# Hansard-T/FHE-Linformer

Measured on AMD Instinct MI355X. Metric: encrypted Linformer-d128 forward ms/sample, lower is better.
Workload: dtype u64

## Files before the change

### fhe-linformer_amd/csrc/context.cpp

```cpp
#include "context.h"
#include <hip/hip_runtime.h>
#include <algorithm>
#include <cstdio>
#include <cstdlib>
#include <cstring>
#include <sys/random.h>
#include <time.h>
#include <cxxabi.h>
#include <dlfcn.h>
#include <execinfo.h>

namespace fhelin {

template <class T>
const T* Context::upload_table(const std::vector<T>& v) {
    void* p = nullptr;
    size_t bytes = std::max<size_t>(v.size() * sizeof(T), 16);
    hip_check(hipMalloc(&p, bytes), "hipMalloc(table)");
    if (!v.empty()) hip_check(hipMemcpy(p, v.data(), v.size() * sizeof(T), hipMemcpyHostToDevice), "hipMemcpy(table)");
    table_allocs.push_back(p);
    return static_cast<const T*>(p);
}
template const u64* Context::upload_table<u64>(const std::vector<u64>&);
template const int* Context::upload_table<int>(const std::vector<int>&);
// ... 53 lines not shown
    try {
        chain = make_prime_chain(p.log_n, p.n_q, p.first_bits, p.scale_bits, p.n_p, p.special_bits);
    } catch (const std::exception& e) {
        throw Error(FHELIN_ERR_ARG, std::string("prime chain: ") + e.what());
    }
    moduli = chain.q;
    moduli.insert(moduli.end(), chain.p.begin(), chain.p.end());
    for (u64 q : moduli)
        if (q >> 60) throw Error(FHELIN_ERR_ARG, "prime chain: a modulus is >= 2^60 (lower scale_bits or first_bits)");
    for (u64 q : moduli) {
        barrett.push_back(h_barrett(q));
        tw.push_back(make_twiddles(q, p.log_n));
    }
    sf_real.assign(p.n_q + 1, 0.0L);
    sf_real[0] = (long double)chain.q[L];
    for (int k = 0; k < L; ++k) sf_real[k + 1] = sf_real[k] * sf_real[k] / (long double)chain.q[L - k];

    pool.fill_word = DevicePool::parse_fill(std::getenv("FHELIN_POOL_FILL"));

    if (p.device < 0) return;

    int ndev = 0;
    if (hipGetDeviceCount(&ndev) != hipSuccess || ndev <= 0)
        throw Error(FHELIN_ERR_NO_DEVICE, "no HIP device visible: the fhe-linformer_amd engine has no CPU fallback");
    if (p.device >= ndev) throw Error(FHELIN_ERR_ARG, "device index out of range");
    hip_check(hipSetDevice(p.device), "hipSetDevice");
    hip_check(hipStreamCreateWithFlags(&stream, hipStreamNonBlocking), "hipStreamCreate");
    main_stream = stream;
    own_stream = true;
    {
        int want = 2;
        if (const char* e = std::getenv("FHELIN_LANES")) want = std::atoi(e);
        n_lanes = std::max(0, std::min(want, DevicePool::MAX_LANES - 1));
        for (int k = 1; k <= n_lanes; ++k) {
            hip_check(hipStreamCreateWithFlags(&lane_stream[k], hipStreamNonBlocking), "hipStreamCreate(lane)");
            hip_check(hipEventCreateWithFlags(&lane_event[k], hipEventDisableTiming), "hipEventCreate(lane)");
        }
        hip_check(hipEventCreateWithFlags(&fork_event, hipEventDisableTiming), "hipEventCreate(fork)");
        pool.lane_stream[0] = main_stream;
        for (int k = 1; k <= n_lanes; ++k) pool.lane_stream[k] = lane_stream[k];
        pool.have_streams = true;
        if (const char* e = std::getenv("FHELIN_ASYNC")) async_lanes = std::atoi(e) != 0;
        if (const char* e = std::getenv("FHELIN_FUSE_MODDOWN")) fuse_moddown = std::atoi(e) != 0;
        if (const char* e = std::getenv("FHELIN_FUSE_FINISH")) fuse_finish = std::atoi(e) != 0;
        if (const char* e = std::getenv("FHELIN_HOST_ENCODE")) host_encode = std::atoi(e) != 0;
        if (const char* e = std::getenv("FHELIN_DEVICE_DECODE")) device_decode = std::atoi(e) != 0;
        if (const char* e = std::getenv("FHELIN_ROT_GATHER")) rot_gather = std::atoi(e) != 0;
        if (const char* e = std::getenv("FHELIN_FUSE_LIFT")) fuse_lift = std::atoi(e) != 0;
        if (const char* e = std::getenv("FHELIN_LDS_DIGITS")) lds_digits = std::atoi(e) != 0;
        if (const char* e = std::getenv("FHELIN_FUSE_ACCP_ROWS")) fuse_accp_rows = std::atoi(e);
        if (const char* e = std::getenv("FHELIN_ACCP_ROWS_MIN_VECS")) accp_rows_min_vecs = std::atoi(e);
        if (const char* e = std::getenv("FHELIN_FUSE_ACCQ_ROWS")) fuse_accq_rows = std::atoi(e);
        if (const char* e = std::getenv("FHELIN_ACCQ_ROWS_MIN_VECS")) accq_rows_min_vecs = std::atoi(e);
        if (const char* e = std::getenv("FHELIN_NTT_TRACE")) trace_small_ntt = std::atoi(e);
        if (const char* e = std::getenv("FHELIN_SCALAR_TRACE")) trace_scalar = std::atoi(e);
        if (const char* e = std::getenv("FHELIN_HOST_WAITS")) trace_waits = std::atoi(e) != 0;
    }
    hip_check(hipEventCreate(&ev_start), "hipEventCreate");
    stage_words = (size_t)2 << p.log_n;
    for (int i = 0; i < STAGE_SLOTS; ++i) {
        hip_check(hipHostMalloc(reinterpret_cast<void**>(&stage_buf[i]), stage_words * sizeof(u64), hipHostMallocDefault), "hipHostMalloc(stage)");
        hip_check(hipEventCreateWithFlags(&stage_ev[i], hipEventDisableTiming), "hipEventCreate(stage)");
    }
    hip_check(hipHostMalloc(reinterpret_cast<void**>(&small_buf), (size_t)SMALL_SLOTS * SMALL_WORDS * sizeof(u64), hipHostMallocDefault), "hipHostMalloc(stage, small)");
    for (int i = 0; i < SMALL_SLOTS; ++i) hip_check(hipEventCreateWithFlags(&small_ev[i], hipEventDisableTiming), "hipEventCreate(stage, small)");
    hip_check(hipEventCreate(&ev_stop), "hipEventCreate");
    has_device = true;

    const int nl = (int)moduli.size();
    {
        std::vector<u64> bar(2 * nl), ninv(8 * nl, 0);
        for (int i = 0; i < nl; ++i) {
            bar[2 * i] = barrett[i].r0;
            bar[2 * i + 1] = barrett[i].r1;
            ninv[8 * i] = tw[i].n_inv;
            ninv[8 * i + 1] = tw[i].n_inv_s;
            ninv[8 * i + 2] = tw[i].w1_n_inv;
            ninv[8 * i + 3] = tw[i].w1_n_inv_s;
            int bits = 0;
            while (bits < 64 && (moduli[i] >> bits)) ++bits;
            if (bits >= 12 && bits <= 60) {
                ninv[8 * i + 4] = (u64)(bits - 10);
                ninv[8 * i + 5] = (u64)((((u128)1) << (bits + 22)) / moduli[i]);
            }
        }
        dt.log_n = p.log_n;
        dt.n_limbs = nl;
        dt.moduli = upload_table(moduli);
        dt.barrett = upload_table(bar);
        {
            std::vector<u64> qi(nl);
            for (int i = 0; i < nl; ++i) {
                u64 x = moduli[i];
                for (int it = 0; it < 6; ++it) x *= 2 - moduli[i] * x;
                qi[i] = x;
            }
            dt.qinv = upload_table(qi);
            std::vector<u64> mr(2 * (size_t)nl);
            for (int i = 0; i < nl; ++i) {
                mr[2 * i] = mont_r(moduli[i]);
                mr[2 * i + 1] = h_shoup(mr[2 * i], moduli[i]);
            }
            dt.mont = upload_table(mr);
        }
        dt.ninv = upload_table(ninv);
        std::vector<u64> f((size_t)nl * 2 * N), g((size_t)nl * 2 * N);
// ... 337 lines not shown
```

### fhe-linformer_amd/csrc/context.h

```cpp
#pragma once
#include <cstdint>
#include <map>
#include <memory>
#include <stdexcept>
#include <string>
#include <unordered_map>
#include <vector>
#include <hip/hip_runtime_api.h>
#include "../../include/fhelin.h"
#include "hostmath.h"
#include "pool.h"
#include "kernels_elem.h"

namespace fhelin {

struct Params {
    int log_n = 16;
    int n_q = 24;
    int first_bits = 55;
    int scale_bits = 52;
    int n_p = 6;
    int special_bits = 60;
    int dnum = 4;
    int log_slots = 14;
// ... 85 lines not shown
    u64* small_buf = nullptr;
    hipEvent_t small_ev[SMALL_SLOTS] = {};
    bool small_used[SMALL_SLOTS] = {};
    int small_next = 0;
    void upload_async(u64* dst, const u64* src, size_t words);

    const u64* d_phatinv = nullptr;
    const u64* d_phatmod = nullptr;
    const u64* d_pinv = nullptr;
    const u64* d_pmod = nullptr;
    const u64* d_qlinv = nullptr;
    const u64* d_qlmod = nullptr;
    std::vector<LevelTables> lvl;
    std::map<u64, const u32*> automorph_maps;

    explicit Context(const Params& p);
    ~Context();
    Context(const Context&) = delete;
    Context& operator=(const Context&) = delete;

    void require_device() const;
    template <class T> T* dalloc(size_t count) { return static_cast<T*>(pool.alloc(count * sizeof(T))); }
    template <class T> Scratch<T> scratch(size_t count) { return Scratch<T>(pool, count); }
    template <class T> const T* upload_table(const std::vector<T>& v);
    int limb_id_q(int i) const { return i; }
    int limb_id_p(int j) const { return L + 1 + j; }
    int digits_at(int ell) const { return (ell + alpha - 1) / alpha; }
    u64 galois_element(long rot_index) const;
    int stride = 1;
    bool stride_explicit = false;
    bool stride_locked = false;
    u64 rot_element(int rot_index) const { return stride == 1 ? galois_element(rot_index) : galois_element((long)stride * rot_index); }
    struct PhysicalScope {
        Context& c;
        int was;
        explicit PhysicalScope(Context& ctx) : c(ctx), was(ctx.stride) { c.stride = 1; }
        ~PhysicalScope() { c.stride = was; }
    };
    const u32* automorph_map(u64 galois);
    const u32* automorph_inverse_of(const u32* map);
    std::map<const u32*, const u32*> automorph_inverse;
    u32 automorph_ginv_of(const u32* map) const;
    std::map<const u32*, u32> automorph_ginv;
    bool fuse_finish = true;
    bool fuse_moddown = false;
    bool host_encode = false;
    bool device_decode = false;
    bool rot_gather = true;
    bool fuse_lift = true;
    int fuse_accp_rows = 1;
    int accp_rows_min_vecs = 0;
    int fuse_accq_rows = 1;
    int accq_rows_min_vecs = 0;
    bool lds_digits = true;
    struct FftDev {
        const u32* rot = nullptr;
        const double* ksi = nullptr;
    };
    std::map<int, FftDev> fft_dev;
    void sync();
    void ntt(const LimbBatch& b, bool inverse, int active = -1) {
        stats.limb_ntt += (u64)(active >= 0 ? active : b.nvec);
        if (trace_small_ntt && b.nvec <= trace_small_ntt) note_small_ntt(b.nvec);
        launch_ntt(dt, b, inverse, stream);
    }
    bool trace_waits = false;
    std::map<std::string, std::pair<u64, u64>> wait_sites;
    void note_wait(const char* site, u64 ns) {
        auto& e = wait_sites[site];
        e.first += 1;
        e.second += ns;
    }
    int trace_small_ntt = 0;
    std::map<std::string, std::pair<u64, u64>> small_ntt_sites;
    void note_small_ntt(int nvec);
    int trace_scalar = 0;
    std::map<std::string, std::pair<u64, u64>> scalar_sites;
    void note_scalar(int nvec);
    void ntt_epilogue(const LimbBatch& b, const NttEpilogue& ep) {
        stats.limb_ntt += (u64)b.nvec;
        if (trace_small_ntt && b.nvec <= trace_small_ntt) note_small_ntt(b.nvec);
        launch_ntt_epilogue(dt, b, ep, stream);
    }
    void ntt_epilogue_product(const LimbBatch& b, const NttEpilogue& ep, const NttProduct& p) {
        stats.limb_ntt += (u64)b.nvec;
        if (trace_small_ntt && b.nvec <= trace_small_ntt) note_small_ntt(b.nvec);
        launch_ntt_epilogue_product(dt, b, ep, p, stream);
    }
};

}
```

### fhe-linformer_amd/csrc/evaluator.cpp

```cpp
#include "evaluator.h"
#include <map>
#include <hip/hip_runtime.h>
#include <cmath>
#include <cstring>

namespace fhelin {

DevBlock::~DevBlock() {
    if (d && ctx) {
        try { ctx->pool.free(d); } catch (...) {}
    }
}
Ciphertext::~Ciphertext() {
    if (async_ev) (void)hipEventDestroy(async_ev);
    if (d && ctx && !block) {
        try { ctx->pool.free(d); } catch (...) {}
    }
}
Encoding::~Encoding() {
    if (ready) (void)hipEventDestroy(ready);
    if (d && ctx) {
        try { ctx->pool.free(d, lanes_ordered); } catch (...) {}
    }
}
// ... 131 lines not shown
}

void Evaluator::keyswitch(const u64* c_ntt, int ell, const EvalKey& key, u64* out, const u64* add0, const u64* add1,
                          const u32* map, const u64* post) {
    keyswitch_batch(1, c_ntt, 0, ell, key, out, 0, add0, add1, 0, map, post, 0);
}

void Evaluator::keyswitch_batch(int B, const u64* c_ntt, size_t c_stride, int ell, const EvalKey& key, u64* out, size_t out_stride,
                                const u64* add0, const u64* add1, size_t add_stride, const u32* map, const u64* post,
                                size_t post_stride) {
    keyswitch_impl(B, nullptr, c_ntt, c_stride, ell, &key, out, out_stride, add0, add1, add_stride, map, post, post_stride);
}

void Evaluator::keyswitch_rows(const KsRows& rows, const u64* c_ntt, size_t c_stride, int ell, u64* out, size_t out_stride,
                               const u64* add0, size_t add_stride) {
    const int B = (int)rows.keys.size();
    if (B < 1) return;
    if (B > KsShape::MAX_ROWS || rows.maps.size() != rows.keys.size()) throw Error(FHELIN_ERR_ARG, "keyswitch_rows: bad row count");
    keyswitch_impl(B, &rows, c_ntt, c_stride, ell, nullptr, out, out_stride, add0, nullptr, add_stride, nullptr, nullptr, 0);
}

void Evaluator::keyswitch_impl(int B, const KsRows* rows, const u64* c_ntt, size_t c_stride, int ell, const EvalKey* key, u64* out,
                               size_t out_stride, const u64* add0, const u64* add1, size_t add_stride, const u32* map, const u64* post,
                               size_t post_stride) {
    c_.require_device();
    if (c_.K < 1) throw Error(FHELIN_ERR_STATE, "hybrid key switching needs at least one special prime");
    if (B < 1) return;
    KsShape sh = ks_shape(ell, B, {c_stride, out_stride, add_stride, post_stride});
    const bool shared = rows && rows->shared_input;
    if (rows) {
        sh.per_row = 1;
        sh.shared_input = shared ? 1 : 0;
        for (int b = 0; b < B; ++b) {
            sh.evk_row[b] = rows->keys[b]->d;
            sh.map_row[b] = rows->maps[b];
        }
    }
    KsShape shu = sh;
    shu.batch = shared ? 1 : B;
    c_.stats.keyswitch += (u64)B;
    c_.stats.keyswitch_limbs += (u64)B * ell;
    const bool identity = !map && !rows;
    const bool gather = !identity && !add1 && rot_in_gather();
    const u64* evk = key ? key->d : nullptr;
    if (gather) evk = set_gather(sh, rows ? rows->keys.data() : &key, rows ? rows->maps.data() : &map, add0, add_stride);
    Scratch<u64> ext = modup(shu, c_ntt, !gather);
    KsAcc acc = inner_product(sh, ext, evk, c_ntt, moddown_tail(gather ? KsOutput::Gathered : identity ? KsOutput::Identity : KsOutput::Scattered));
    moddown(acc, gather ? KsOut{out, nullptr, nullptr, post} : KsOut{out, add0, add1, post, map});
    launch_ok("keyswitch");
}


KsShape Evaluator::ks_shape(int ell, int batch, const KsStrides& st) const {
    return KsShape{ell, c_.K, c_.alpha, c_.lvl[ell].beta, c_.L + 1, batch, st.c, st.out, st.add, st.post};
}

Evaluator::KsTail Evaluator::moddown_tail(KsOutput o) const {
    const bool rows = o == KsOutput::Gathered || (o == KsOutput::Identity && (c_.fuse_moddown || c_.fuse_finish)) ||
                      (o == KsOutput::Scattered && c_.fuse_moddown) || (o == KsOutput::MergedSum && c_.fuse_finish && c_.rot_gather);
    return rows ? KsTail::RowPass : KsTail::Finish;
}

const u64* Evaluator::set_gather(KsShape& sh, const EvalKey* const* keys, const u32* const* maps, const u64* c0, size_t c0_stride) {
    const u64* evk = nullptr;
    sh.gather = 1;
    if (sh.per_row) {
        for (int b = 0; b < (sh.row_mod ? sh.row_mod : sh.batch); ++b) {
            sh.evk_row[b] = permuted(*keys[b], maps[b]);
            sh.ginv_row[b] = c_.automorph_ginv_of(maps[b]);
        }
    } else {
        evk = permuted(*keys[0], maps[0]);
        sh.map_row[0] = maps[0];
        sh.ginv = c_.automorph_ginv_of(maps[0]);
    }
    if (c0) {
        sh.gsrc = c0;
        sh.gsrc_stride = c0_stride;
        sh.gsrc_pmod = c_.d_pmod;
    }
    return evk;
}

Scratch<u64> Evaluator::modup(const KsShape& up, const u64* src, bool times_r2, int group2, size_t group2_stride) {
    const size_t N = c_.N;
    const int n = up.batch, ell = up.ell, nt = ell + c_.K;
    const LevelTables& lt = c_.lvl[ell];
    Scratch<u64> cc = c_.scratch<u64>((size_t)n * ell * N);
    {
        LimbBatch ib{cc, n * ell, nullptr, 0, ell, src};
        if (n > 1 && up.c_stride != (size_t)ell * N) {
            ib.src_group = ell;
            ib.src_group_stride = up.c_stride;
        }
        if (group2 > 0) {
            ib.src_group2 = group2;
            ib.src_group2_stride = group2_stride;
        }
        c_.ntt(ib, true);
    }
    Scratch<u64> ext = c_.scratch<u64>((size_t)n * lt.beta * nt * N);
    launch_modup_conv(c_.dt, up, ext, cc, src, lt.up_hatinv, times_r2 ? lt.up_hatmod_r2 : lt.up_hatmod, c_.stream);
    LimbBatch eb{ext, n * lt.beta * nt, lt.ext_limb_tab, 0, 1};
    eb.tab_len = lt.beta * nt;
    eb.lazy_out = true;
    c_.ntt(eb, false, n * (lt.beta * nt - ell));
    return ext;
// ... 1875 lines not shown
```

### fhe-linformer_amd/csrc/kernels_elem.h

```cpp
#pragma once
#include "kernels.h"

namespace fhelin {

struct ScalarSet {
    u64 v[128];
};

void launch_ew_mul(const DeviceTables& t, u64* out, const u64* a, const u64* b, int nvec, int b_mod, int limb_first, int limb_count, hipStream_t s);
void launch_ew_add(const DeviceTables& t, u64* out, const u64* a, const u64* b, int nvec, int b_mod, int limb_first, int limb_count, hipStream_t s);
void launch_ew_sub(const DeviceTables& t, u64* out, const u64* a, const u64* b, int nvec, int b_mod, int limb_first, int limb_count, hipStream_t s);
void launch_ew_muladd(const DeviceTables& t, u64* out, const u64* acc, const u64* a, const u64* b, int nvec, int b_mod, int limb_first,
                      int limb_count, hipStream_t s);
void launch_ew_neg(const DeviceTables& t, u64* out, const u64* a, int nvec, int limb_first, int limb_count, hipStream_t s);
void launch_ew_scalar(const DeviceTables& t, u64* out, const u64* a, const ScalarSet& sc, int nvec, int limb_first, int limb_count, hipStream_t s,
                      int in_limbs = 0);
void launch_ew_addscalar(const DeviceTables& t, u64* out, const u64* a, const ScalarSet& sc, int nvec, int limb_first, int limb_count, hipStream_t s,
                         int add_vecs = -1);
struct LinComb {
    static constexpr int MAX_TERMS = 32;
    int n = 0;
    int vecs = 0;
    const u64* a[MAX_TERMS];
};
// ... 81 lines not shown
};
void launch_ew_dot_groups(const DeviceTables& t, const EwDotGroups& d, hipStream_t s);
struct EwCyclic {
    static constexpr int PERIOD = 32;
    int n = 0, ell = 0;
    const u64* a[PERIOD];
    const u64* m[PERIOD];
    u64* out[PERIOD];
};
void launch_ew_cyclic_dot(const DeviceTables& t, const EwCyclic& d, hipStream_t s);
struct EwWindow {
    static constexpr int W = 32;
    int ell = 0, accumulate = 0;
    u32 cur_mask = 0, prev_mask = 0;
    const u64* cur[W];
    const u64* prev[W];
    const u64* m[W];
    u64* out[W];
};
void launch_ew_window_dot(const DeviceTables& t, const EwWindow& d, hipStream_t s);

struct KsShape {
    int ell;
    int k;
    int alpha;
    int beta;
    int L1;
    int batch = 1;
    size_t c_stride = 0;
    size_t out_stride = 0;
    size_t add_stride = 0;
    size_t post_stride = 0;
    static constexpr int MAX_ROWS = 16;
    int per_row = 0;
    int shared_input = 0;
    int row_mod = 0;
    const u64* evk_row[MAX_ROWS] = {};
    const u32* map_row[MAX_ROWS] = {};
    static constexpr int MAX_ROT = 7;
    int n_rot = 0;
    const u64* evk_rot[MAX_ROT] = {};
    const u32* map_rot[MAX_ROT] = {};
    size_t rot_ext_stride = 0;
    size_t rot_input_stride = 0;
    int lds_digits = 0;
    size_t ext_batch_stride = 0;
    const u64* gsrc = nullptr;
    size_t gsrc_stride = 0;
    const u64* gsrc_pmod = nullptr;
    int gather = 0;
    u32 ginv = 0;
    u32 ginv_row[MAX_ROWS] = {};
    int tch = 16;
    int accp_limbs = 0;
    int accp_rows = 0;
    int accq_rows = 0;
};
struct NttProduct {
    KsShape sh;
    const u64* ext = nullptr;
    const u64* evk = nullptr;
    int multi = 0;
    const u64* c_ntt = nullptr;
};
void launch_ntt_rows_product(const DeviceTables& t, const LimbBatch& b, const NttProduct& p, hipStream_t s);
void launch_ntt_epilogue_product(const DeviceTables& t, const LimbBatch& b, const NttEpilogue& ep, const NttProduct& p, hipStream_t s);
void launch_ntt_cols_inverse(const DeviceTables& t, const LimbBatch& b, hipStream_t s);
void launch_modup_conv(const DeviceTables& t, const KsShape& sh, u64* ext, const u64* cc, const u64* c_ntt, const u64* hatinv,
                       const u64* hatmod, hipStream_t s);
void launch_ks_inner(const DeviceTables& t, const KsShape& sh, u64* accQ, u64* accP, const u64* ext, const u64* evk, const u64* c_ntt,
                     hipStream_t s);
void launch_ks_inner_multi(const DeviceTables& t, const KsShape& sh, u64* accQ, u64* accP, const u64* ext, const u64* c_ntt,
                           hipStream_t s);
void launch_fold_key(const DeviceTables& t, u64* out, const u64* key, const u32* map, const u64* V, int nvec, hipStream_t s);
struct HoistAdd {
    int n_rot = 0;
    const u64* v[KsShape::MAX_ROT + 1] = {};
    const u32* map[KsShape::MAX_ROT] = {};
    u64* acc = nullptr;
    const u64* pmod = nullptr;
};
void launch_hoist_addends(const DeviceTables& t, const KsShape& sh, const HoistAdd& h, u64* pre, const u64* ct, hipStream_t s);
struct LtStep {
    static constexpr int MAX_G = 4;
    const u64* key;
    const u32* map;
    const u64* v[MAX_G];
    u32 mask;
    u32 pad;
};
struct LtDot {
    static constexpr int MAX_STEPS = 32;
    const LtStep* steps = nullptr;
    int n_steps = 0;
    int n_groups = 0;
    int g0 = 0, groups = 0;
    const u64* pmod = nullptr;
};
void launch_ks_inner_dot(const DeviceTables& t, const KsShape& sh, const LtDot& ld, u64* accQ, u64* accP, const u64* ext, const u64* c0,
                         const u64* c1, hipStream_t s);
void launch_moddown_conv(const DeviceTables& t, const KsShape& sh, u64* conv, const u64* accP, const u64* phatinv, const u64* phatmod,
                         hipStream_t s);
void launch_affine_acc(const DeviceTables& t, const KsShape& sh, u64* accQ, const u64* d, const u64* sub, const ScalarSet& cst, int has_cst, int f,
                       const u64* pmod, hipStream_t s);
void launch_moddown_rescale_conv(const DeviceTables& t, const KsShape& sh, u64* conv, const u64* accP, const u64* top, const u64* hatinv,
                                 const u64* hatmod, const u64* mmod, hipStream_t s);
// ... 16 lines not shown
```

### fhe-linformer_amd/csrc/kernels_ks.hip

```cpp
#include <hip/hip_runtime.h>
#include <cstdlib>
#include "kernels.h"
#include "kernels_elem.h"

namespace fhelin {
namespace {

typedef u64 u64x2 __attribute__((ext_vector_type(2)));

__device__ __forceinline__ Barrett load_barrett(const DeviceTables& t, int limb) {
    Barrett b;
    b.q = t.moduli[limb];
    b.r0 = t.barrett[2 * limb];
    b.r1 = t.barrett[2 * limb + 1];
    return b;
}

constexpr int TCH = 16;

template <int MAXA, bool FULL>
__device__ __forceinline__ void modup_body(const DeviceTables& t, const KsShape& sh, u64* __restrict__ ext, const u64* __restrict__ cc,
                                           const u64* __restrict__ hatinv, const u64* __restrict__ hatmod, int j, int lo, int cnt, size_t n) {
    const size_t N = (size_t)1 << t.log_n;
    const int nt = sh.ell + sh.k;
    u32 y0[MAXA], y1[MAXA];
#pragma unroll
    for (int i = 0; i < MAXA; ++i) {
        if (FULL || i < cnt) {
            const int li = lo + i;
            split30(mul_shoup(cc[(size_t)li * N + n], hatinv[2 * li], hatinv[2 * li + 1], t.moduli[li]), y0[i], y1[i]);
        } else {
            y0[i] = y1[i] = 0;
        }
    }
    u64* dst = ext + (size_t)j * nt * N + n;
    const int t0 = blockIdx.z * sh.tch, t1 = min(nt, t0 + sh.tch);
    for (int tt = t0; tt < t1; ++tt) {
        if (tt >= lo && tt < lo + cnt) continue;
        const int limb = tt < sh.ell ? tt : sh.L1 + (tt - sh.ell);
        const u64 qt = t.moduli[limb], qti = t.qinv[limb];
        u64 slo = 0, shi = 0;
#pragma unroll
        for (int i0 = 0; i0 < MAXA; i0 += 8) {
            Acc30 acc = {0, 0, 0};
#pragma unroll
            for (int i = i0; i < i0 + 8 && i < MAXA; ++i)
                if (FULL || i < cnt) {
                    const u64 h = hatmod[(size_t)(lo + i) * nt + tt];
                    mac30(acc, y0[i], y1[i], (u32)h, (u32)(h >> 32));
                }
            acc30_flush(acc, slo, shi);
        }
        dst[(size_t)tt * N] = redc128(slo, shi, qt, qti);
    }
}

template <int MAXA>
__global__ __launch_bounds__(256) void modup_conv_kernel(DeviceTables t, KsShape sh, u64* __restrict__ ext, const u64* __restrict__ cc, const u64* __restrict__ c_ntt,
                                                         const u64* __restrict__ hatinv, const u64* __restrict__ hatmod) {
    const int bi = blockIdx.y / sh.beta, j = blockIdx.y % sh.beta;
    const size_t N = (size_t)1 << t.log_n;
    const size_t n = (size_t)blockIdx.x * 256 + threadIdx.x;
    const int lo = j * sh.alpha;
    const int cnt = min(sh.alpha, sh.ell - lo);
    const int nt = sh.ell + sh.k;
    cc += (size_t)bi * sh.ell * N;
    ext += (size_t)bi * sh.beta * nt * N;
    (void)c_ntt;
    if (cnt == MAXA)
        modup_body<MAXA, true>(t, sh, ext, cc, hatinv, hatmod, j, lo, cnt, n);
    else
        modup_body<MAXA, false>(t, sh, ext, cc, hatinv, hatmod, j, lo, cnt, n);
}

struct KsBlock {
    int bx, bi, tt;
};
__device__ __forceinline__ KsBlock ks_block(const KsShape& sh, int rows = 0) {
    const unsigned nx = gridDim.x, nblk = gridDim.x * gridDim.y;
    const unsigned nb = rows ? (unsigned)rows : (unsigned)sh.batch;
    unsigned b = blockIdx.y * nx + blockIdx.x;
    if ((nblk & 7) == 0) b = (b & 7) * (nblk >> 3) + (b >> 3);
    KsBlock k;
    k.bi = (int)(b % nb);
    k.bx = (int)((b / nb) % nx);
    k.tt = (int)(b / (nb * nx));
    return k;
}

__device__ __forceinline__ u32 sel_mask(u32 a, u32 b, unsigned long long mask) {
    u32 r;
    asm("v_cndmask_b32_e64 %0, %1, %2, %3" : "=v"(r) : "v"(a), "v"(b), "s"(mask));
    return r;
}

template <bool GATHER>
__global__ __launch_bounds__(256) void ks_inner_kernel(DeviceTables t, KsShape sh, u64* __restrict__ accQ, u64* __restrict__ accP, const u64* __restrict__ ext,
                                                       const u64* __restrict__ evk, const u64* __restrict__ c_ntt) {
    const int nt = sh.ell + sh.k;
    const KsBlock kb_ = ks_block(sh);
    const int bi = kb_.bi, tt = kb_.tt;
    const int limb = tt < sh.ell ? tt : sh.L1 + (tt - sh.ell);
    const int in = sh.row_mod ? bi / sh.row_mod : bi;
    const int ri = sh.per_row ? (sh.row_mod ? bi % sh.row_mod : bi) : 0;
    if (sh.row_mod) {
        ext += (size_t)in * sh.ext_batch_stride;
        c_ntt += (size_t)in * sh.c_stride;
        evk = sh.evk_row[bi % sh.row_mod];
    } else {
        if (!sh.shared_input) {
            ext += (size_t)bi * sh.beta * nt * ((size_t)1 << t.log_n);
            c_ntt += (size_t)bi * sh.c_stride;
        }
        if (sh.per_row) evk = sh.evk_row[bi];
    }
    const int own = tt < sh.ell ? tt / sh.alpha : -1;
    accQ += (size_t)bi * 2 * sh.ell * ((size_t)1 << t.log_n);
    const int pk = sh.accp_limbs ? sh.accp_limbs : sh.k;
    accP += (size_t)bi * 2 * pk * ((size_t)1 << t.log_n);
    const Barrett br = load_barrett(t, limb);
    const size_t row = ((size_t)1 << t.log_n) >> 1;
    const size_t n2 = (size_t)kb_.bx * 256 + threadIdx.x;
    const size_t kstride = (size_t)(sh.L1 + sh.k) * row;
    const u64x2* E = reinterpret_cast<const u64x2*>(ext);
    const u64x2* K = reinterpret_cast<const u64x2*>(evk);
// ... 363 lines not shown
    u32 z0[MAXK], z1[MAXK];
#pragma unroll
    for (int p = 0; p < MAXK; ++p) {
        if (FULL || p < sh.k) {
            const u64 m = t.moduli[sh.L1 + p];
            u64 x = accP[((size_t)c * sh.k + p) * N + n];
            if constexpr (SIGNED) x = neg && x ? m - x : x;
            split30(mul_shoup(x, phatinv[2 * p], phatinv[2 * p + 1], m), z0[p], z1[p]);
        } else {
            z0[p] = z1[p] = 0;
        }
    }
    u64* dst = conv + (size_t)c * sh.ell * N + n;
    const int t0 = blockIdx.z * sh.tch, t1 = min(sh.ell, t0 + sh.tch);
    for (int tt = t0; tt < t1; ++tt) {
        const u64 qt = t.moduli[tt], qti = t.qinv[tt];
        u64 slo = 0, shi = 0;
#pragma unroll
        for (int p0 = 0; p0 < MAXK; p0 += 8) {
            Acc30 acc = {0, 0, 0};
#pragma unroll
            for (int p = p0; p < p0 + 8 && p < MAXK; ++p)
                if (FULL || p < sh.k) {
                    const u64 h = phatmod[(size_t)p * sh.L1 + tt];
                    mac30(acc, z0[p], z1[p], (u32)h, (u32)(h >> 32));
                }
            acc30_flush(acc, slo, shi);
        }
        u64 r = redc128(slo, shi, qt, qti);
        if constexpr (SIGNED) r = neg && r ? qt - r : r;
        dst[(size_t)tt * N] = r;
    }
}

template <int MAXK, bool SIGNED = false>
__global__ __launch_bounds__(256) void moddown_conv_kernel(DeviceTables t, KsShape sh, u64* __restrict__ conv, const u64* __restrict__ accP, const u64* __restrict__ phatinv,
                                                           const u64* __restrict__ phatmod) {
    const int bi = blockIdx.y >> 1, c = blockIdx.y & 1;
    const size_t N = (size_t)1 << t.log_n;
    const size_t n = (size_t)blockIdx.x * 256 + threadIdx.x;
    accP += (size_t)bi * 2 * sh.k * N;
    conv += (size_t)bi * 2 * sh.ell * N;
    bool neg = false;
    if constexpr (SIGNED) {
        const u32 gi = sh.per_row ? sh.ginv_row[sh.row_mod ? bi % sh.row_mod : bi] : sh.ginv;
        neg = ((gi * (u32)n) & (u32)(2 * N - 1)) >= (u32)N;
    }
    if (sh.k == MAXK)
        moddown_body<MAXK, true, SIGNED>(t, sh, conv, accP, phatinv, phatmod, c, n, neg);
    else
        moddown_body<MAXK, false, SIGNED>(t, sh, conv, accP, phatinv, phatmod, c, n, neg);
}

__global__ __launch_bounds__(256) void moddown_finish_kernel(DeviceTables t, KsShape sh, u64* __restrict__ out, const u64* __restrict__ accQ, const u64* __restrict__ conv,
                                                             const u64* __restrict__ pinv, const u64* __restrict__ add0, const u64* __restrict__ add1, const u32* __restrict__ map,
                                                             const u64* __restrict__ post) {
    const int bi = blockIdx.y / (2 * sh.ell), v = blockIdx.y % (2 * sh.ell);
    const int c = v / sh.ell, tt = v % sh.ell;
    const u64 q = t.moduli[tt];
    const u64 w = pinv[2 * tt], ws = pinv[2 * tt + 1];
    const size_t N = (size_t)1 << t.log_n;
    const size_t j = ((size_t)blockIdx.x * 256 + threadIdx.x) * 2;
    accQ += (size_t)bi * 2 * sh.ell * N;
    conv += (size_t)bi * 2 * sh.ell * N;
    out += (size_t)bi * sh.out_stride;
    const u64* add = c == 0 ? add0 : add1;
    if (add) add += (size_t)(sh.row_mod ? bi / sh.row_mod : bi) * sh.add_stride;
    if (post) post += (size_t)bi * sh.post_stride;
    if (sh.per_row) map = sh.map_row[sh.row_mod ? bi % sh.row_mod : bi];
    u64x2 r;
    if (map) {
        const u32 m0 = map[j], m1 = map[j + 1];
        r.x = mul_shoup(sub_mod(accQ[(size_t)v * N + m0], conv[(size_t)v * N + m0], q), w, ws, q);
        r.y = mul_shoup(sub_mod(accQ[(size_t)v * N + m1], conv[(size_t)v * N + m1], q), w, ws, q);
        if (add) {
            r.x = add_mod(r.x, add[(size_t)tt * N + m0], q);
            r.y = add_mod(r.y, add[(size_t)tt * N + m1], q);
        }
    } else {
        const u64x2 a = reinterpret_cast<const u64x2*>(accQ)[((size_t)v * N + j) >> 1];
        const u64x2 b = reinterpret_cast<const u64x2*>(conv)[((size_t)v * N + j) >> 1];
        r.x = mul_shoup(sub_mod(a.x, b.x, q), w, ws, q);
        r.y = mul_shoup(sub_mod(a.y, b.y, q), w, ws, q);
        if (add) {
            const u64x2 d = reinterpret_cast<const u64x2*>(add)[((size_t)tt * N + j) >> 1];
            r.x = add_mod(r.x, d.x, q);
            r.y = add_mod(r.y, d.y, q);
        }
    }
    if (post) {
        const u64x2 p = reinterpret_cast<const u64x2*>(post)[((size_t)v * N + j) >> 1];
        r.x = add_mod(r.x, p.x, q);
        r.y = add_mod(r.y, p.y, q);
    }
    if (sh.gsrc && !sh.gsrc_pmod && c == 0) {
        const u64* __restrict__ g = sh.gsrc + (size_t)bi * sh.gsrc_stride + (size_t)tt * N;
        for (int rr = 0; rr < sh.n_rot; ++rr) {
            const u64* __restrict__ gr = g + (size_t)rr * sh.rot_input_stride;
            const u32* __restrict__ mr = sh.map_rot[rr];
            const u32 m0 = mr ? mr[j] : (u32)j;
            const u64x2 gp = reinterpret_cast<const u64x2*>(gr)[m0 >> 1];
            r.x = add_mod(r.x, (m0 & 1) ? gp.y : gp.x, q);
            r.y = add_mod(r.y, (m0 & 1) ? gp.x : gp.y, q);
        }
    }
    reinterpret_cast<u64x2*>(out)[((size_t)v * N + j) >> 1] = r;
// ... 219 lines not shown
                                                                         const u64* __restrict__ phatmod, const u64* __restrict__ pinv,
                                                                         const u64* __restrict__ pmod, const u64* __restrict__ qlm) {
    const int bi = blockIdx.y >> 1;
    const size_t N = (size_t)1 << t.log_n;
    const size_t n = (size_t)blockIdx.x * 256 + threadIdx.x;
    const bool f2 = (f2_mask >> bi) & 1;
    const u64* src = accP + (size_t)blockIdx.y * (sh.k + 1) * N + n;
    u64* dst = conv + (size_t)blockIdx.y * (sh.ell - 1) * N + n;
    if (sh.k == MAXK)
        moddown_exact_body<MAXK, true>(t, sh, f2, dst, src, phatinv, phatmod, pinv, pmod, qlm);
    else
        moddown_exact_body<MAXK, false>(t, sh, f2, dst, src, phatinv, phatmod, pinv, pmod, qlm);
}

__global__ __launch_bounds__(256) void moddown_rescale_finish_kernel(DeviceTables t, KsShape sh, u64* __restrict__ out, const u64* __restrict__ accQ,
                                                                     const u64* __restrict__ conv, const u64* __restrict__ minv) {
    const int e1 = sh.ell - 1;
    const int bi = blockIdx.y / (2 * e1), v = blockIdx.y % (2 * e1);
    const int c = v / e1, tt = v % e1;
    const u64 q = t.moduli[tt];
    const u64 w = minv[2 * tt], ws = minv[2 * tt + 1];
    const size_t row = ((size_t)1 << t.log_n) >> 1;
    const size_t n2 = (size_t)blockIdx.x * 256 + threadIdx.x;
    const u64x2 a = reinterpret_cast<const u64x2*>(accQ)[(((size_t)bi * 2 + c) * sh.ell + tt) * row + n2];
    const u64x2 b = reinterpret_cast<const u64x2*>(conv)[(((size_t)bi * 2 + c) * e1 + tt) * row + n2];
    u64x2 r;
    r.x = mul_shoup(sub_mod(a.x, b.x, q), w, ws, q);
    r.y = mul_shoup(sub_mod(a.y, b.y, q), w, ws, q);
    reinterpret_cast<u64x2*>(out + (size_t)bi * sh.out_stride)[(size_t)v * row + n2] = r;
}

}

void launch_fold_key(const DeviceTables& t, u64* out, const u64* key, const u32* map, const u64* V, int nvec, hipStream_t s) {
    hipLaunchKernelGGL(fold_key_kernel, dim3((1u << t.log_n) / 512, (unsigned)nvec), dim3(256), 0, s, t, out, key, map, V);
}
void launch_hoist_addends(const DeviceTables& t, const KsShape& sh, const HoistAdd& h, u64* pre, const u64* ct, hipStream_t s) {
    hipLaunchKernelGGL(hoist_addends_kernel, dim3((1u << t.log_n) / 512, (unsigned)(sh.batch * 2 * sh.ell)), dim3(256), 0, s, t, sh, h, pre, ct);
}

void launch_affine_acc(const DeviceTables& t, const KsShape& sh, u64* accQ, const u64* d, const u64* sub, const ScalarSet& cst, int has_cst, int f,
                       const u64* pmod, hipStream_t s) {
    hipLaunchKernelGGL(affine_acc_kernel, dim3((1u << t.log_n) / 512, (unsigned)(sh.batch * 2 * sh.ell)), dim3(256), 0, s, t, sh, accQ, d, sub, cst,
                       has_cst, f, pmod);
}
static int conv_tch(unsigned planes, int targets) {
    static const int force = [] {
        const char* e = std::getenv("FHELIN_CONV_CHUNKS");
        return e ? std::atoi(e) : 0;
    }();
    if (force || planes < 2048u) return TCH;
    return targets > TCH ? targets : TCH;
}
void launch_moddown_rescale_conv(const DeviceTables& t, const KsShape& sh_in, u64* conv, const u64* accP, const u64* top, const u64* hatinv,
                                 const u64* hatmod, const u64* mmod, hipStream_t s) {
    KsShape sh = sh_in;
    const unsigned nx = (1u << t.log_n) / 256;
    sh.tch = conv_tch(nx * (unsigned)(sh.batch * 2), sh.ell - 1);
    dim3 g(nx, (unsigned)(sh.batch * 2), (unsigned)((sh.ell - 1 + sh.tch - 1) / sh.tch));
    hipLaunchKernelGGL(moddown_rescale_conv_kernel, g, dim3(256), 0, s, t, sh, conv, accP, top, hatinv, hatmod, mmod);
}
void launch_affine_acc_items(const DeviceTables& t, const KsShape& sh, const AffineItems& it, u64* accQ, u64* accP, const u64* d,
                             const u64* consts, const u64* pmod, hipStream_t s) {
    dim3 g((1u << t.log_n) / 512, (unsigned)(sh.batch * 2 * sh.ell));
    hipLaunchKernelGGL(affine_acc_items_kernel, g, dim3(256), 0, s, t, sh, it, accQ, accP, d, consts, pmod);
}
void launch_moddown_rescale_exact_conv(const DeviceTables& t, const KsShape& sh_in, u32 f2, u64* conv, const u64* accP, const u64* phatinv,
                                       const u64* phatmod, const u64* pinv, const u64* pmod, const u64* qlm, hipStream_t s) {
    KsShape sh = sh_in;
    const unsigned nx = (1u << t.log_n) / 256;
    sh.tch = conv_tch(nx * (unsigned)(sh.batch * 2), sh.ell - 1);
    dim3 g(nx, (unsigned)(sh.batch * 2), (unsigned)((sh.ell - 1 + sh.tch - 1) / sh.tch));
#define FHELIN_MDX_CASE(K) case K: hipLaunchKernelGGL((moddown_rescale_exact_conv_kernel<K>), g, dim3(256), 0, s, t, sh, f2, conv, accP, phatinv, phatmod, pinv, pmod, qlm); break;
    switch (sh.k) {
        FHELIN_MDX_CASE(1) FHELIN_MDX_CASE(2) FHELIN_MDX_CASE(3) FHELIN_MDX_CASE(4)
        FHELIN_MDX_CASE(5) FHELIN_MDX_CASE(6) FHELIN_MDX_CASE(7) FHELIN_MDX_CASE(8)
        default: hipLaunchKernelGGL((moddown_rescale_exact_conv_kernel<16>), g, dim3(256), 0, s, t, sh, f2, conv, accP, phatinv, phatmod, pinv, pmod, qlm); break;
    }
#undef FHELIN_MDX_CASE
}
void launch_moddown_rescale_finish(const DeviceTables& t, const KsShape& sh, u64* out, const u64* accQ, const u64* conv, const u64* minv,
                                   hipStream_t s) {
    dim3 g((1u << t.log_n) / 512, (unsigned)(sh.batch * 2 * (sh.ell - 1)));
    hipLaunchKernelGGL(moddown_rescale_finish_kernel, g, dim3(256), 0, s, t, sh, out, accQ, conv, minv);
}

void launch_modup_conv(const DeviceTables& t, const KsShape& sh_in, u64* ext, const u64* cc, const u64* c_ntt, const u64* hatinv,
                       const u64* hatmod, hipStream_t s) {
    KsShape sh = sh_in;
    const unsigned nx = (1u << t.log_n) / 256;
    sh.tch = conv_tch(nx * (unsigned)(sh.batch * sh.beta), sh.ell + sh.k);
    dim3 g(nx, (unsigned)(sh.batch * sh.beta), (unsigned)((sh.ell + sh.k + sh.tch - 1) / sh.tch));
#define FHELIN_MODUP_CASE(A) case A: hipLaunchKernelGGL((modup_conv_kernel<A>), g, dim3(256), 0, s, t, sh, ext, cc, c_ntt, hatinv, hatmod); break;
    switch (sh.alpha) {
        FHELIN_MODUP_CASE(1) FHELIN_MODUP_CASE(2) FHELIN_MODUP_CASE(3) FHELIN_MODUP_CASE(4)
        FHELIN_MODUP_CASE(5) FHELIN_MODUP_CASE(6) FHELIN_MODUP_CASE(7) FHELIN_MODUP_CASE(8)
        default: hipLaunchKernelGGL((modup_conv_kernel<16>), g, dim3(256), 0, s, t, sh, ext, cc, c_ntt, hatinv, hatmod); break;
    }
#undef FHELIN_MODUP_CASE
}
void launch_ks_inner(const DeviceTables& t, const KsShape& sh, u64* accQ, u64* accP, const u64* ext, const u64* evk, const u64* c_ntt,
                     hipStream_t s) {
    dim3 g((1u << t.log_n) / 512, (unsigned)(sh.batch * (sh.accp_rows ? sh.ell : sh.ell + sh.k)));
    if (sh.gather)
        hipLaunchKernelGGL(ks_inner_kernel<true>, g, dim3(256), 0, s, t, sh, accQ, accP, ext, evk, c_ntt);
    else
        hipLaunchKernelGGL(ks_inner_kernel<false>, g, dim3(256), 0, s, t, sh, accQ, accP, ext, evk, c_ntt);
}
void launch_ks_inner_multi(const DeviceTables& t, const KsShape& sh, u64* accQ, u64* accP, const u64* ext, const u64* c_ntt,
                           hipStream_t s) {
    static const int pair_rows = [] { const char* e = std::getenv("FHELIN_KS_ROW_PAIRS"); return e ? std::atoi(e) : 1; }();
    const bool stage = sh.lds_digits && sh.rot_ext_stride == 0 && sh.beta <= 4;
    const int nt = sh.accp_rows ? sh.ell : sh.ell + sh.k;
    if (pair_rows && sh.batch >= 2) {
        dim3 g((1u << t.log_n) / 512, (unsigned)(((sh.batch + 1) / 2) * nt));
        if (stage)
            hipLaunchKernelGGL((ks_inner_multi_kernel<true, 2>), g, dim3(256), 0, s, t, sh, accQ, accP, ext, c_ntt);
        else
            hipLaunchKernelGGL((ks_inner_multi_kernel<false, 2>), g, dim3(256), 0, s, t, sh, accQ, accP, ext, c_ntt);
        return;
    }
    dim3 g((1u << t.log_n) / 512, (unsigned)(sh.batch * nt));
    if (stage)
        hipLaunchKernelGGL((ks_inner_multi_kernel<true, 1>), g, dim3(256), 0, s, t, sh, accQ, accP, ext, c_ntt);
    else
        hipLaunchKernelGGL((ks_inner_multi_kernel<false, 1>), g, dim3(256), 0, s, t, sh, accQ, accP, ext, c_ntt);
}
void launch_ks_inner_dot(const DeviceTables& t, const KsShape& sh, const LtDot& ld, u64* accQ, u64* accP, const u64* ext, const u64* c0,
                         const u64* c1, hipStream_t s) {
    dim3 g((1u << t.log_n) / 512, (unsigned)(sh.batch * (sh.ell + sh.k)));
    if (ld.n_groups == 1)
        hipLaunchKernelGGL(ks_inner_dot_kernel<1>, g, dim3(256), 0, s, t, sh, ld, accQ, accP, ext, c0, c1);
    else if (ld.n_groups == 2)
        hipLaunchKernelGGL(ks_inner_dot_kernel<2>, g, dim3(256), 0, s, t, sh, ld, accQ, accP, ext, c0, c1);
    else
        hipLaunchKernelGGL((ks_inner_dot_kernel<LtStep::MAX_G>), g, dim3(256), 0, s, t, sh, ld, accQ, accP, ext, c0, c1);
}
void launch_moddown_conv(const DeviceTables& t, const KsShape& sh_in, u64* conv, const u64* accP, const u64* phatinv, const u64* phatmod,
                         hipStream_t s) {
    KsShape sh = sh_in;
    const unsigned nx = (1u << t.log_n) / 256;
    sh.tch = conv_tch(nx * (unsigned)(2 * sh.batch), sh.ell);
    dim3 g(nx, (unsigned)(2 * sh.batch), (unsigned)((sh.ell + sh.tch - 1) / sh.tch));
#define FHELIN_MODDOWN_CASE(K, S) case K: hipLaunchKernelGGL((moddown_conv_kernel<K, S>), g, dim3(256), 0, s, t, sh, conv, accP, phatinv, phatmod); break;
#define FHELIN_MODDOWN_SWITCH(S)                                                                                                                \
    switch (sh.k) {                                                                                                                             \
        FHELIN_MODDOWN_CASE(1, S) FHELIN_MODDOWN_CASE(2, S) FHELIN_MODDOWN_CASE(3, S) FHELIN_MODDOWN_CASE(4, S)                                 \
        FHELIN_MODDOWN_CASE(5, S) FHELIN_MODDOWN_CASE(6, S) FHELIN_MODDOWN_CASE(7, S) FHELIN_MODDOWN_CASE(8, S)                                 \
        default: hipLaunchKernelGGL((moddown_conv_kernel<16, S>), g, dim3(256), 0, s, t, sh, conv, accP, phatinv, phatmod); break;              \
    }
    if (sh.gather) {
        FHELIN_MODDOWN_SWITCH(true)
    } else {
        FHELIN_MODDOWN_SWITCH(false)
    }
#undef FHELIN_MODDOWN_SWITCH
#undef FHELIN_MODDOWN_CASE
}
void launch_moddown_finish(const DeviceTables& t, const KsShape& sh, u64* out, const u64* accQ, const u64* conv, const u64* pinv,
                           const u64* add0, const u64* add1, const u32* map, const u64* post, hipStream_t s) {
    dim3 g((1u << t.log_n) / 512, (unsigned)(sh.batch * 2 * sh.ell));
    hipLaunchKernelGGL(moddown_finish_kernel, g, dim3(256), 0, s, t, sh, out, accQ, conv, pinv, add0, add1, map, post);
}

}
```

Before: 216.9.

## Process two coefficients per thread in modup and moddown base conversion kernels

Adds pair variants of the modup and moddown base-conversion kernels. Each thread loads two adjacent coefficients as a 128-bit vector and reuses each target modulus's constants and hatmod row for both, halving the grid's x dimension. Constants for the next target are prefetched while the current one is computed. The pair path is on by default when alpha or k is at most 8 and the buffers are 16-byte aligned. This cuts per-coefficient table loads and widens memory accesses, at the cost of more registers per thread and possibly lower occupancy.

```diff
diff --git a/fhe-linformer_amd/csrc/context.cpp b/fhe-linformer_amd/csrc/context.cpp
--- a/fhe-linformer_amd/csrc/context.cpp
+++ b/fhe-linformer_amd/csrc/context.cpp
@@ -129,6 +129,7 @@
         if (const char* e = std::getenv("FHELIN_ACCP_ROWS_MIN_VECS")) accp_rows_min_vecs = std::atoi(e);
         if (const char* e = std::getenv("FHELIN_FUSE_ACCQ_ROWS")) fuse_accq_rows = std::atoi(e);
         if (const char* e = std::getenv("FHELIN_ACCQ_ROWS_MIN_VECS")) accq_rows_min_vecs = std::atoi(e);
+        if (const char* e = std::getenv("FHELIN_CONV_PAIRS")) conv_pairs = std::atoi(e) != 0;
         if (const char* e = std::getenv("FHELIN_NTT_TRACE")) trace_small_ntt = std::atoi(e);
         if (const char* e = std::getenv("FHELIN_SCALAR_TRACE")) trace_scalar = std::atoi(e);
         if (const char* e = std::getenv("FHELIN_HOST_WAITS")) trace_waits = std::atoi(e) != 0;
diff --git a/fhe-linformer_amd/csrc/context.h b/fhe-linformer_amd/csrc/context.h
--- a/fhe-linformer_amd/csrc/context.h
+++ b/fhe-linformer_amd/csrc/context.h
@@ -161,6 +161,7 @@
     int accp_rows_min_vecs = 0;
     int fuse_accq_rows = 1;
     int accq_rows_min_vecs = 0;
+    bool conv_pairs = true;
     bool lds_digits = true;
     struct FftDev {
         const u32* rot = nullptr;
diff --git a/fhe-linformer_amd/csrc/evaluator.cpp b/fhe-linformer_amd/csrc/evaluator.cpp
--- a/fhe-linformer_amd/csrc/evaluator.cpp
+++ b/fhe-linformer_amd/csrc/evaluator.cpp
@@ -207,7 +207,9 @@
 
 
 KsShape Evaluator::ks_shape(int ell, int batch, const KsStrides& st) const {
-    return KsShape{ell, c_.K, c_.alpha, c_.lvl[ell].beta, c_.L + 1, batch, st.c, st.out, st.add, st.post};
+    KsShape sh{ell, c_.K, c_.alpha, c_.lvl[ell].beta, c_.L + 1, batch, st.c, st.out, st.add, st.post};
+    sh.conv_pairs = c_.conv_pairs ? 1 : 0;
+    return sh;
 }
 
 Evaluator::KsTail Evaluator::moddown_tail(KsOutput o) const {
diff --git a/fhe-linformer_amd/csrc/kernels_elem.h b/fhe-linformer_amd/csrc/kernels_elem.h
--- a/fhe-linformer_amd/csrc/kernels_elem.h
+++ b/fhe-linformer_amd/csrc/kernels_elem.h
@@ -157,6 +157,7 @@
     u32 ginv = 0;
     u32 ginv_row[MAX_ROWS] = {};
     int tch = 16;
+    int conv_pairs = 1;
     int accp_limbs = 0;
     int accp_rows = 0;
     int accq_rows = 0;
diff --git a/fhe-linformer_amd/csrc/kernels_ks.hip b/fhe-linformer_amd/csrc/kernels_ks.hip
--- a/fhe-linformer_amd/csrc/kernels_ks.hip
+++ b/fhe-linformer_amd/csrc/kernels_ks.hip
@@ -1,4 +1,5 @@
 #include <hip/hip_runtime.h>
+#include <cstdint>
 #include <cstdlib>
 #include "kernels.h"
 #include "kernels_elem.h"
@@ -71,6 +72,90 @@
         modup_body<MAXA, true>(t, sh, ext, cc, hatinv, hatmod, j, lo, cnt, n);
     else
         modup_body<MAXA, false>(t, sh, ext, cc, hatinv, hatmod, j, lo, cnt, n);
+}
+
+template <int MAXS, bool FULL>
+__device__ __forceinline__ u64x2 conv_pair_target(const u32 (&y0)[2][MAXS], const u32 (&y1)[2][MAXS], const u64 (&h)[MAXS], int cnt, u64 qt,
+                                                  u64 qti) {
+    static_assert(MAXS <= 8, "one Acc30 holds at most 8 products");
+    Acc30 a = {0, 0, 0}, b = {0, 0, 0};
+#pragma unroll
+    for (int i = 0; i < MAXS; ++i)
+        if (FULL || i < cnt) {
+            mac30(a, y0[0][i], y1[0][i], (u32)h[i], (u32)(h[i] >> 32));
+            mac30(b, y0[1][i], y1[1][i], (u32)h[i], (u32)(h[i] >> 32));
+        }
+    u64 alo = 0, ahi = 0, blo = 0, bhi = 0;
+    acc30_flush(a, alo, ahi);
+    acc30_flush(b, blo, bhi);
+    u64x2 r;
+    r.x = redc128(alo, ahi, qt, qti);
+    r.y = redc128(blo, bhi, qt, qti);
+    return r;
+}
+
+template <int MAXA, bool FULL>
+__device__ __forceinline__ void modup_pair_body(const DeviceTables& t, const KsShape& sh, u64* __restrict__ ext, const u64* __restrict__ cc,
+                                                const u64* __restrict__ hatinv, const u64* __restrict__ hatmod, int j, int lo, int cnt, size_t n2) {
+    const size_t row = ((size_t)1 << t.log_n) >> 1;
+    const int nt = sh.ell + sh.k;
+    const u64x2* C = reinterpret_cast<const u64x2*>(cc);
+    u64x2 x[MAXA];
+#pragma unroll
+    for (int i = 0; i < MAXA; ++i) x[i] = C[(size_t)(lo + (FULL || i < cnt ? i : 0)) * row + n2];
+    u32 y0[2][MAXA], y1[2][MAXA];
+#pragma unroll
+    for (int i = 0; i < MAXA; ++i) {
+        const bool live = FULL || i < cnt;
+        const int li = lo + (live ? i : 0);
+        const u64 w = hatinv[2 * li], ws = hatinv[2 * li + 1], q = t.moduli[li];
+        const u64 a = mul_shoup(x[i].x, w, ws, q), b = mul_shoup(x[i].y, w, ws, q);
+        split30(live ? a : 0, y0[0][i], y1[0][i]);
+        split30(live ? b : 0, y0[1][i], y1[1][i]);
+    }
+    u64x2* dst = reinterpret_cast<u64x2*>(ext + (size_t)j * nt * ((size_t)1 << t.log_n)) + n2;
+    const int t0 = blockIdx.z * sh.tch, t1 = min(nt, t0 + sh.tch);
+    struct Consts {
+        u64 h[MAXA], qt, qti;
+    };
+    auto consts = [&](int tt) {
+        Consts c;
+        const int limb = tt < sh.ell ? tt : sh.L1 + (tt - sh.ell);
+        c.qt = t.moduli[limb];
+        c.qti = t.qinv[limb];
+#pragma unroll
+        for (int i = 0; i < MAXA; ++i) c.h[i] = hatmod[(size_t)(lo + (FULL || i < cnt ? i : 0)) * nt + tt];
+        return c;
+    };
+#pragma unroll 1
+    for (int r = 0; r < 2; ++r) {
+        const int a = r ? max(t0, lo + cnt) : t0, b = r ? t1 : min(t1, lo);
+        if (a >= b) continue;
+        Consts cur = consts(a);
+#pragma unroll 1
+        for (int tt = a; tt < b; ++tt) {
+            const Consts nxt = consts(min(tt + 1, b - 1));
+            dst[(size_t)tt * row] = conv_pair_target<MAXA, FULL>(y0, y1, cur.h, cnt, cur.qt, cur.qti);
+            cur = nxt;
+        }
+    }
+}
+
+template <int MAXA>
+__global__ __launch_bounds__(256) void modup_conv_pair_kernel(DeviceTables t, KsShape sh, u64* __restrict__ ext, const u64* __restrict__ cc,
+                                                              const u64* __restrict__ hatinv, const u64* __restrict__ hatmod) {
+    const int bi = blockIdx.y / sh.beta, j = blockIdx.y % sh.beta;
+    const size_t N = (size_t)1 << t.log_n;
+    const size_t n2 = (size_t)blockIdx.x * 256 + threadIdx.x;
+    const int lo = j * sh.alpha;
+    const int cnt = min(sh.alpha, sh.ell - lo);
+    const int nt = sh.ell + sh.k;
+    cc += (size_t)bi * sh.ell * N;
+    ext += (size_t)bi * sh.beta * nt * N;
+    if (cnt == MAXA)
+        modup_pair_body<MAXA, true>(t, sh, ext, cc, hatinv, hatmod, j, lo, cnt, n2);
+    else
+        modup_pair_body<MAXA, false>(t, sh, ext, cc, hatinv, hatmod, j, lo, cnt, n2);
 }
 
 struct KsBlock {
@@ -540,6 +625,63 @@
         moddown_body<MAXK, false, SIGNED>(t, sh, conv, accP, phatinv, phatmod, c, n, neg);
 }
 
+template <int K, bool SIGNED>
+__global__ __launch_bounds__(256) void moddown_conv_pair_kernel(DeviceTables t, KsShape sh, u64* __restrict__ conv, const u64* __restrict__ accP,
+                                                                const u64* __restrict__ phatinv, const u64* __restrict__ phatmod) {
+    const int bi = blockIdx.y >> 1, c = blockIdx.y & 1;
+    const size_t row = ((size_t)1 << t.log_n) >> 1;
+    const size_t n2 = (size_t)blockIdx.x * 256 + threadIdx.x;
+    const u64x2* A = reinterpret_cast<const u64x2*>(accP) + ((size_t)bi * 2 + c) * K * row + n2;
+    u64x2 x[K];
+#pragma unroll
+    for (int p = 0; p < K; ++p) x[p] = A[(size_t)p * row];
+    bool neg0 = false, neg1 = false;
+    if constexpr (SIGNED) {
+        const u32 gi = sh.per_row ? sh.ginv_row[sh.row_mod ? bi % sh.row_mod : bi] : sh.ginv;
+        const u32 m2 = (u32)(4 * row - 1), N = (u32)(2 * row);
+        neg0 = ((gi * (u32)(2 * n2)) & m2) >= N;
+        neg1 = ((gi * (u32)(2 * n2 + 1)) & m2) >= N;
+    }
+    u32 z0[2][K], z1[2][K];
+#pragma unroll
+    for (int p = 0; p < K; ++p) {
+        const u64 m = t.moduli[sh.L1 + p], w = phatinv[2 * p], ws = phatinv[2 * p + 1];
+        u64 a = x[p].x, b = x[p].y;
+        if constexpr (SIGNED) {
+            a = neg0 && a ? m - a : a;
+            b = neg1 && b ? m - b : b;
+        }
+        split30(mul_shoup(a, w, ws, m), z0[0][p], z1[0][p]);
+        split30(mul_shoup(b, w, ws, m), z0[1][p], z1[1][p]);
+    }
+    u64x2* dst = reinterpret_cast<u64x2*>(conv) + ((size_t)bi * 2 + c) * sh.ell * row + n2;
+    const int t0 = blockIdx.z * sh.tch, t1 = min(sh.ell, t0 + sh.tch);
+    struct Consts {
+        u64 h[K], qt, qti;
+    };
+    auto consts = [&](int tt) {
+        Consts cs;
+        cs.qt = t.moduli[tt];
+        cs.qti = t.qinv[tt];
+#pragma unroll
+        for (int p = 0; p < K; ++p) cs.h[p] = phatmod[(size_t)p * sh.L1 + tt];
+        return cs;
+    };
+    if (t0 >= t1) return;
+    Consts cur = consts(t0);
+#pragma unroll 1
+    for (int tt = t0; tt < t1; ++tt) {
+        const Consts nxt = consts(min(tt + 1, t1 - 1));
+        u64x2 r = conv_pair_target<K, true>(z0, z1, cur.h, K, cur.qt, cur.qti);
+        if constexpr (SIGNED) {
+            r.x = neg0 && r.x ? cur.qt - r.x : r.x;
+            r.y = neg1 && r.y ? cur.qt - r.y : r.y;
+        }
+        dst[(size_t)tt * row] = r;
+        cur = nxt;
+    }
+}
+
 __global__ __launch_bounds__(256) void moddown_finish_kernel(DeviceTables t, KsShape sh, u64* __restrict__ out, const u64* __restrict__ accQ, const u64* __restrict__ conv,
                                                              const u64* __restrict__ pinv, const u64* __restrict__ add0, const u64* __restrict__ add1, const u32* __restrict__ map,
                                                              const u64* __restrict__ post) {
@@ -865,6 +1007,9 @@
     if (force || planes < 2048u) return TCH;
     return targets > TCH ? targets : TCH;
 }
+static bool conv_in_pairs(const KsShape& sh, int sources, const void* in, const void* out) {
+    return sh.conv_pairs && sources <= 8 && ((reinterpret_cast<uintptr_t>(in) | reinterpret_cast<uintptr_t>(out)) & 15u) == 0;
+}
 void launch_moddown_rescale_conv(const DeviceTables& t, const KsShape& sh_in, u64* conv, const u64* accP, const u64* top, const u64* hatinv,
                                  const u64* hatmod, const u64* mmod, hipStream_t s) {
     KsShape sh = sh_in;
@@ -904,6 +1049,16 @@
     const unsigned nx = (1u << t.log_n) / 256;
     sh.tch = conv_tch(nx * (unsigned)(sh.batch * sh.beta), sh.ell + sh.k);
     dim3 g(nx, (unsigned)(sh.batch * sh.beta), (unsigned)((sh.ell + sh.k + sh.tch - 1) / sh.tch));
+    if (conv_in_pairs(sh, sh.alpha, cc, ext)) {
+        g.x = nx / 2;
+#define FHELIN_MODUP_CASE(A) case A: hipLaunchKernelGGL((modup_conv_pair_kernel<A>), g, dim3(256), 0, s, t, sh, ext, cc, hatinv, hatmod); break;
+        switch (sh.alpha) {
+            FHELIN_MODUP_CASE(1) FHELIN_MODUP_CASE(2) FHELIN_MODUP_CASE(3) FHELIN_MODUP_CASE(4)
+            FHELIN_MODUP_CASE(5) FHELIN_MODUP_CASE(6) FHELIN_MODUP_CASE(7) FHELIN_MODUP_CASE(8)
+        }
+#undef FHELIN_MODUP_CASE
+        return;
+    }
 #define FHELIN_MODUP_CASE(A) case A: hipLaunchKernelGGL((modup_conv_kernel<A>), g, dim3(256), 0, s, t, sh, ext, cc, c_ntt, hatinv, hatmod); break;
     switch (sh.alpha) {
         FHELIN_MODUP_CASE(1) FHELIN_MODUP_CASE(2) FHELIN_MODUP_CASE(3) FHELIN_MODUP_CASE(4)
@@ -955,6 +1110,19 @@
     const unsigned nx = (1u << t.log_n) / 256;
     sh.tch = conv_tch(nx * (unsigned)(2 * sh.batch), sh.ell);
     dim3 g(nx, (unsigned)(2 * sh.batch), (unsigned)((sh.ell + sh.tch - 1) / sh.tch));
+    if (conv_in_pairs(sh, sh.k, accP, conv)) {
+        g.x = nx / 2;
+#define FHELIN_MODDOWN_CASE(K) case K:                                                                                                    \
+        if (sh.gather) hipLaunchKernelGGL((moddown_conv_pair_kernel<K, true>), g, dim3(256), 0, s, t, sh, conv, accP, phatinv, phatmod);  \
+        else hipLaunchKernelGGL((moddown_conv_pair_kernel<K, false>), g, dim3(256), 0, s, t, sh, conv, accP, phatinv, phatmod);           \
+        break;
+        switch (sh.k) {
+            FHELIN_MODDOWN_CASE(1) FHELIN_MODDOWN_CASE(2) FHELIN_MODDOWN_CASE(3) FHELIN_MODDOWN_CASE(4)
+            FHELIN_MODDOWN_CASE(5) FHELIN_MODDOWN_CASE(6) FHELIN_MODDOWN_CASE(7) FHELIN_MODDOWN_CASE(8)
+        }
+#undef FHELIN_MODDOWN_CASE
+        return;
+    }
 #define FHELIN_MODDOWN_CASE(K, S) case K: hipLaunchKernelGGL((moddown_conv_kernel<K, S>), g, dim3(256), 0, s, t, sh, conv, accP, phatinv, phatmod); break;
 #define FHELIN_MODDOWN_SWITCH(S)                                                                                                                \
     switch (sh.k) {                                                                                                                             \
```

Result: no change. 215.2 (median of 6 runs) (-0.8%).
